# UmaimaKhan01/SkyEye-Aerial-Object-Detection-using-Yolo

Hardware: AMD Instinct MI355X
Metric: frames/sec @1280x1280 + p50 latency, skyeye_s 1-GPU and skyeye_l 8-GPU (higher is better)
Workload: dtype bf16

## Files before the change

skyeye-aerial-object-detection-using-yolo_amd/csrc/engine.cpp:

```cpp
#include "../../include/skyeye_hip.h"
#include "sky_kernels.h"
#include "build_hash.h"

#include <cstddef>
#include <hip/hip_runtime.h>

#include <algorithm>
#include <cmath>
#include <cstdio>
#include <cstring>
#include <map>
#include <memory>
#include <stdexcept>
#include <string>
#include <vector>

namespace sky {

struct Error : std::runtime_error {
    int code;
    Error(int c, const std::string& m) : std::runtime_error(m), code(c) {}
};

#define SKY_HIP(expr)                                                                                   \
// ... 1911 lines not shown

int sky_num_params(const sky_handle* h) { return h ? (int)h->e.spec.size() : 0; }

int sky_param_info(const sky_handle* h, int index, const char** name, int32_t* ndim, int64_t shape[4])
{
    if (!h || index < 0 || index >= (int)h->e.spec.size()) return SKY_ERR_INVALID;
    const ParamSpec& p = h->e.spec[index];
    if (name) *name = p.name.c_str();
    if (ndim) *ndim = (int32_t)p.shape.size();
    if (shape) for (size_t i = 0; i < 4; ++i) shape[i] = i < p.shape.size() ? p.shape[i] : 0;
    return SKY_OK;
}

int sky_load_weights(sky_handle* h, const sky_tensor_desc* descs, int n)
{
    if (!h) return SKY_ERR_INVALID;
    return guarded(h, [&] {
        for (int i = 0; i < n; ++i) {
            const sky_tensor_desc& d = descs[i];
            if (!d.name || !d.data) throw Error(SKY_ERR_INVALID, "sky_load_weights: null name/data");
            HostTensor t;
            for (int k = 0; k < d.ndim; ++k) t.shape.push_back(d.shape[k]);
            t.data.assign((const float*)d.data, (const float*)d.data + t.numel());
            h->e.weights[d.name] = std::move(t);
        }
        h->e.weights_dirty = true;
    });
}

int sky_plan(sky_handle* h, int n_inputs, const sky_buffer* in)
{
    if (!h) return SKY_ERR_INVALID;
    return guarded(h, [&] {
        if (n_inputs < 1 || n_inputs > SKY_MAX_IO) throw Error(SKY_ERR_INVALID, "sky_plan: bad input count");
        int ndev = 0;
        if (hipGetDeviceCount(&ndev) != hipSuccess || ndev == 0) throw Error(SKY_ERR_NO_DEVICE, "no HIP device visible: the HIP engine cannot run (there is no CPU fallback)");
        DeviceGuard dg(h->e.cfg.device);
        const Geometry g = geometry_of(n_inputs, in);
        plan(h->e, g);
        h->geom = g;
    });
}

int sky_num_outputs(const sky_handle* h) { return h ? (int)h->e.out_info.size() : 0; }

int sky_output_info(const sky_handle* h, int index, int32_t* ndim, int64_t shape[5])
{
    if (!h || index < 0 || index >= (int)h->e.out_info.size()) return SKY_ERR_INVALID;
    const IoInfo& io = h->e.out_info[index];
    if (ndim) *ndim = io.ndim;
    if (shape) for (int i = 0; i < 5; ++i) shape[i] = io.shape[i];
    return SKY_OK;
}

static void check_forward(sky_handle* h, int n_inputs, const sky_buffer* inputs, int n_outputs, const sky_buffer* outputs)
{
    if (!h->e.planned) throw Error(SKY_ERR_STATE, "sky_forward before sky_plan");
    if (h->e.weights_dirty) throw Error(SKY_ERR_STATE, "weights changed after sky_plan: call sky_plan again");
    if (!h->e.calibrated) throw Error(SKY_ERR_STATE, "fp8 engine without activation scales: call sky_calibrate (or sky_scales_write) after sky_plan");
    if (n_inputs != h->geom.n) throw Error(SKY_ERR_SHAPE, "sky_forward: input count differs from the plan");
    if (n_outputs != (int)h->e.out_info.size()) throw Error(SKY_ERR_SHAPE, "sky_forward: expected " + std::to_string(h->e.out_info.size()) + " outputs");
    for (int i = 0; i < n_inputs; ++i) {
        if (!inputs[i].data) throw Error(SKY_ERR_INVALID, "sky_forward: null input");
        for (int k = 0; k < h->geom.ndim[i]; ++k)
            if (inputs[i].shape[k] != h->geom.shape[i][k]) throw Error(SKY_ERR_SHAPE, "sky_forward: input shape differs from the plan");
    }
    std::vector<char> optional(n_outputs, 0);
    for (const Op& op : h->e.ops)
        if (op.kind == OP_CONV && op.head && op.raw_ext >= 16 && op.raw_ext - 16 < n_outputs) optional[op.raw_ext - 16] = 1;
    for (int i = 0; i < n_outputs; ++i) {
        if (!outputs[i].data && !optional[i]) throw Error(SKY_ERR_INVALID, "sky_forward: null output");
        if (!outputs[i].data) continue;
        const IoInfo& oi = h->e.out_info[i];
        bool same = outputs[i].ndim == oi.ndim;
        for (int k = 0; same && k < oi.ndim; ++k) same = outputs[i].shape[k] == oi.shape[k];
        if (!same) throw Error(SKY_ERR_SHAPE, "sky_forward: output " + std::to_string(i) + " has another shape than the plan's (sky_output_info)");
    }
}

int sky_forward(sky_handle* h, int n_inputs, const sky_buffer* inputs, int n_outputs, const sky_buffer* outputs, void* stream)
{
    if (!h) return SKY_ERR_INVALID;
    return guarded(h, [&] {
        check_forward(h, n_inputs, inputs, n_outputs, outputs);
        DeviceGuard dg(h->e.cfg.device);
        run(h->e, inputs, n_inputs, outputs, n_outputs, (hipStream_t)stream);
    });
}

int sky_time_forward(sky_handle* h, int n_inputs, const sky_buffer* inputs, int n_outputs, const sky_buffer* outputs, void* stream,
                     int iters, float* ms_per_iter)
{
    if (!h) return SKY_ERR_INVALID;
    return guarded(h, [&] {
        check_forward(h, n_inputs, inputs, n_outputs, outputs);
        DeviceGuard dg(h->e.cfg.device);
        hipStream_t s = (hipStream_t)stream;
        hipEvent_t e0, e1;
        SKY_HIP(hipEventCreate(&e0));
        SKY_HIP(hipEventCreate(&e1));
        SKY_HIP(hipEventRecord(e0, s));
        for (int i = 0; i < iters; ++i) run(h->e, inputs, n_inputs, outputs, n_outputs, s);
        SKY_HIP(hipEventRecord(e1, s));
        SKY_HIP(hipEventSynchronize(e1));
        float ms = 0;
        SKY_HIP(hipEventElapsedTime(&ms, e0, e1));
        (void)hipEventDestroy(e0);
        (void)hipEventDestroy(e1);
        if (ms_per_iter) *ms_per_iter = ms / (float)std::max(iters, 1);
    });
}

int sky_profile_forward(sky_handle* h, int n_inputs, const sky_buffer* inputs, int n_outputs, const sky_buffer* outputs, void* stream,
                        int iters, int max_ops, float* ms_per_op, double* flops_per_op, int32_t* tag_per_op, int32_t* n_ops)
{
    if (!h) return SKY_ERR_INVALID;
    return guarded(h, [&] {
        check_forward(h, n_inputs, inputs, n_outputs, outputs);
        DeviceGuard dg(h->e.cfg.device);
        const int n = (int)h->e.ops.size();
        if (n_ops) *n_ops = n;
        if (n > max_ops) throw Error(SKY_ERR_INVALID, "sky_profile_forward: max_ops too small");
        hipStream_t s = (hipStream_t)stream;
        std::vector<hipEvent_t> ev(n + 1);
        for (auto& e : ev) SKY_HIP(hipEventCreate(&e));
        std::vector<double> acc(n, 0.0);
        for (int it = 0; it < iters; ++it) {
            run(h->e, inputs, n_inputs, outputs, n_outputs, s, ev.data());
            SKY_HIP(hipEventSynchronize(ev[n]));
            for (int i = 0; i < n; ++i) {
                float ms = 0;
                SKY_HIP(hipEventElapsedTime(&ms, ev[i], ev[i + 1]));
                acc[i] += ms;
            }
        }
        for (auto& e : ev) (void)hipEventDestroy(e);
        for (int i = 0; i < n; ++i) {
            const Op& op = h->e.ops[i];
            if (ms_per_op) ms_per_op[i] = (float)(acc[i] / std::max(iters, 1));
            if (flops_per_op) flops_per_op[i] = op.flops;
            if (tag_per_op) tag_per_op[i] = (int)op.kind * 10000 + (op.kind == OP_CONV || op.kind == OP_IMPORT ? op.variant : 0);
        }
    });
}

int sky_op_info(const sky_handle* h, int index, char* text, int text_len)
{
    if (!h || !text || index < 0 || index >= (int)h->e.ops.size()) return SKY_ERR_INVALID;
    static const char* names[] = {"import", "export", "conv", "maxpool5", "upsample", "ca_reduce", "ca_mlp", "sa_stats", "sa_gate", "scale", "decode", "layernorm", "attention", "cla", "export_tokens"};
    const Op& op = h->e.ops[index];
    if (op.kind == OP_CONV)
        snprintf(text, text_len, "conv %dx%d s%d %d->%d in %dx%dx%d out %dx%d ld %d/%d%s%s%s %s%d", op.ks, op.ks, op.stride, op.cin, op.cout,
                 op.in.B, op.in.H, op.in.W, op.Ho, op.Wo, op.in.ld, op.out.ld, op.res.valid() ? (op.in2_cin ? " +res in2" : " +res") : (op.in2_cin ? " in2" : ""), op.up2 ? " up2" : "",
                 op.head ? " head" : "", op.variant >= 9000 ? "fused-into-previous" : op.variant >= 8500 ? "csp-stage-fused-" : op.variant >= 8000 ? "stem+stride2-fused-" : op.variant == 1628 ? "cv3+head/" : op.variant == 3256 ? "gemm1x1/" : op.variant == 7128 ? "bneck" : op.variant == 7256 ? "bneck128x2/" : op.variant == 7257 ? "bneck128x2-fp8/" : op.variant == 7065 ? "bneck64x3/" : op.variant == 7066 ? "bneck64x4-fp8/" : op.variant >= 7000 ? "halo-cv1+3x3-" : op.variant >= 6000 ? "halo-s2-" : op.variant >= 5000 ? "halo-narrow" : op.variant >= 4600 ? "deep3x3/" : op.variant >= 4000 ? "halo" : op.variant >= 3000 ? "ring" : op.variant >= 2000 ? "stream" : op.variant >= 1500 ? "head-stream" : "tile", op.variant % (op.variant >= 1500 && op.variant < 2000 ? 500 : 1000));
    else
        snprintf(text, text_len, "%s in %dx%dx%dx%d out C%d", names[op.kind], op.in.B, op.in.H, op.in.W, op.in.C, op.out.C);
    if (h->e.opts) {
        const size_t n = strlen(text);
        if ((int)n + 16 < text_len) snprintf(text + n, text_len - n, " opts=0x%x", h->e.opts);
    }
    return SKY_OK;
}

int sky_op_bytes(const sky_handle* h, int index, double* bytes)
{
    if (!h || !bytes || index < 0 || index >= (int)h->e.ops.size()) return SKY_ERR_INVALID;
    const Op& op = h->e.ops[index];
    const int es = h->e.esize();
    auto sz = [&](const TV& t, int esz) { return (t.buf >= 0 || t.ext >= 0) && t.B ? (double)t.B * t.H * t.W * t.C * (t.buf >= 0 ? dtype_size(t.dt) : esz) : 0.0; };
    double b = sz(op.in, es) + sz(op.out, es) + sz(op.res, es) + sz(op.in2, es);
    if (op.kind == OP_CONV && op.head) b += 2.0 * op.in.B * op.Ho * op.Wo * (double)op.cout * 4;
    if (op.kind == OP_IMPORT) b += (double)op.out.B * op.src_c * op.src_h * op.src_w;
    *bytes = b;
    return SKY_OK;
}

int sky_op_io_bytes(const sky_handle* h, int index, int with_raw, double* read_bytes, double* written_bytes)
{
    if (!h || !read_bytes || !written_bytes || index < 0 || index >= (int)h->e.ops.size()) return SKY_ERR_INVALID;
    const Op& op = h->e.ops[index];
    const int es = h->e.esize();
    auto sz = [&](const TV& t, int esz) { return (t.buf >= 0 || t.ext >= 0) && t.B ? (double)t.B * t.H * t.W * t.C * (t.buf >= 0 ? dtype_size(t.dt) : esz) : 0.0; };
    double r = sz(op.in, es) + sz(op.res, es) + sz(op.in2, es), w = sz(op.out, es);
    if (op.kind == OP_CONV && op.head) w += (with_raw ? 2.0 : 1.0) * op.in.B * op.Ho * op.Wo * (double)op.cout * 4;
    if (op.kind == OP_IMPORT) r = (double)op.out.B * op.src_c * op.src_h * op.src_w;
    *read_bytes = r;
    *written_bytes = w;
    return SKY_OK;
}

int sky_plan_stats(const sky_handle* h, double* flops, double* activation_bytes, double* weight_bytes, int32_t* launches)
{
    if (!h || !h->e.planned) return SKY_ERR_STATE;
    if (flops) *flops = h->e.flops;
    if (activation_bytes) *activation_bytes = h->e.act_bytes;
    if (weight_bytes) *weight_bytes = h->e.weight_bytes;
    if (launches) *launches = (int32_t)h->e.ops.size();
    return SKY_OK;
}

int sky_num_packed(const sky_handle* h)
{
    if (!h || !h->e.planned) return SKY_ERR_STATE;
    return (int)h->e.convs.size();
}

int sky_packed_info(const sky_handle* h, int i, sky_packed_desc* out)
{
    if (!h || !out) return SKY_ERR_INVALID;
    if (!h->e.planned) return SKY_ERR_STATE;
    if (i < 0 || i >= (int)h->e.convs.size()) return SKY_ERR_INVALID;
    const DevConv& d = h->e.convs[i];
    memset(out, 0, sizeof(*out));
    snprintf(out->name, sizeof(out->name), "%s", d.name.c_str());
    out->rows = d.rows; out->cout = d.cout; out->kpad = d.Kpad; out->kernel_size = d.ks; out->cin = d.cin;
    out->dtype = d.cdt;
    return SKY_OK;
}

int sky_packed_read(sky_handle* h, int i, void* weights_host, size_t weight_bytes, float* bias_host, size_t bias_count)
{
    if (!h) return SKY_ERR_INVALID;
    return guarded(h, [&] {
        if (!h->e.planned) throw Error(SKY_ERR_STATE, "sky_packed_read: plan the graph first (weights are packed at plan time)");
        DeviceGuard dg(h->e.cfg.device);
        if (i < 0 || i >= (int)h->e.convs.size()) throw Error(SKY_ERR_INVALID, "sky_packed_read: index out of range");
        const DevConv& d = h->e.convs[i];
        if (weights_host) {
            if (weight_bytes < d.bytes) throw Error(SKY_ERR_INVALID, "sky_packed_read: weight buffer too small");
            SKY_HIP(hipMemcpy(weights_host, d.w, d.bytes, hipMemcpyDeviceToHost));
        }
        if (bias_host) {
            if (bias_count < (size_t)d.rows) throw Error(SKY_ERR_INVALID, "sky_packed_read: bias buffer too small");
            SKY_HIP(hipMemcpy(bias_host, d.bias, (size_t)d.rows * sizeof(float), hipMemcpyDeviceToHost));
        }
    });
}

int sky_packed_scales(sky_handle* h, int i, float* scales_host, size_t count)
{
    if (!h) return SKY_ERR_INVALID;
    return guarded(h, [&] {
        if (!h->e.planned) throw Error(SKY_ERR_STATE, "sky_packed_scales: plan the graph first");
        if (i < 0 || i >= (int)h->e.convs.size() || !scales_host) throw Error(SKY_ERR_INVALID, "sky_packed_scales: bad argument");
        const DevConv& d = h->e.convs[i];
        if (count < (size_t)d.rows) throw Error(SKY_ERR_INVALID, "sky_packed_scales: buffer too small");
        for (int r = 0; r < d.rows; ++r) scales_host[r] = d.w_scale.empty() ? (float)(1.0 / (double)d.pre) : d.w_scale[r];
    });
}

int sky_calibrate(sky_handle* h, int n_inputs, const sky_buffer* inputs, void* stream)
{
    if (!h) return SKY_ERR_INVALID;
    return guarded(h, [&] {
        if (n_inputs != h->geom.n) throw Error(SKY_ERR_SHAPE, "sky_calibrate: input count differs from the plan");
        for (int i = 0; i < n_inputs; ++i)
            if (!inputs[i].data) throw Error(SKY_ERR_INVALID, "sky_calibrate: null input");
        DeviceGuard dg(h->e.cfg.device);
        calibrate(h->e, n_inputs, inputs, (hipStream_t)stream);
    });
}

int sky_num_scales(const sky_handle* h) { return h && h->e.planned ? (int)h->e.bufs.size() : 0; }

int sky_scales_read(sky_handle* h, float* scales_host, int n)
{
    if (!h) return SKY_ERR_INVALID;
    return guarded(h, [&] {
        if (!h->e.planned || !scales_host || n < (int)h->e.bufs.size()) throw Error(SKY_ERR_INVALID, "sky_scales_read: plan first / buffer too small");
        for (size_t i = 0; i < h->e.bufs.size(); ++i) {
            TV t; t.buf = (int)i; t.dt = h->e.bufs[i].dt;
            scales_host[i] = tv_scale(h->e, t);
        }
    });
}

int sky_scales_write(sky_handle* h, const float* scales_host, int n)
{
    if (!h) return SKY_ERR_INVALID;
    return guarded(h, [&] {
        if (!h->e.planned || !scales_host || n != (int)h->e.bufs.size()) throw Error(SKY_ERR_INVALID, "sky_scales_write: plan first; one scale per workspace buffer (sky_num_scales)");
        if (h->e.dtype != SKY_FP8) throw Error(SKY_ERR_STATE, "sky_scales_write: only the fp8 engine has activation scales");
        for (int i = 0; i < n; ++i)
            if (!(scales_host[i] > 0.0f)) throw Error(SKY_ERR_INVALID, "sky_scales_write: scales must be positive");
        DeviceGuard dg(h->e.cfg.device);
        for (int i = 0; i < n; ++i) {
            int r = i;
            while (h->e.bufs[r].tie >= 0) r = h->e.bufs[r].tie;
            if (h->e.bufs[i].dt == SKY_FP8) h->e.bufs[r].scale = scales_host[i];
        }
        apply_scales(h->e);
        h->e.calibrated = true;
    });
}

int sky_nms(sky_handle* h, const float* det, int B, int N, int nc, const sky_nms_params* p, float* out, int32_t* counts, void* stream)
{
    if (!h) return SKY_ERR_INVALID;
    return guarded(h, [&] {
        if (!det || !p || !out || !counts) throw Error(SKY_ERR_INVALID, "sky_nms: null argument");
        const bool has_strides = p->struct_size == sizeof(sky_nms_params);
        if (!has_strides && p->struct_size != offsetof(sky_nms_params, out_image_stride))
            throw Error(SKY_ERR_INVALID, "sky_nms: sky_nms_params size mismatch (ABI)");
        if (B < 1 || N < 1 || nc < 1) throw Error(SKY_ERR_SHAPE, "sky_nms: bad geometry");
        if (p->max_detections < 1 || p->max_detections > 4096) throw Error(SKY_ERR_INVALID, "sky_nms: max_detections must be in [1, 4096]");
        if (p->n_classes > 64) throw Error(SKY_ERR_INVALID, "sky_nms: at most 64 class filters");
        DeviceGuard dg(h->e.cfg.device);
// ... 129 lines not shown
```

skyeye-aerial-object-detection-using-yolo_amd/csrc/k_conv_halo.hip:

```cpp
#include "sky_kernels.h"

#ifndef SKY_HALO_VGPR
#define SKY_HALO_VGPR 256
#endif

#include "conv_frag.h"

#ifdef SKY_EXPERIMENTS
#define SKY_DBG(a) ((a).dbg)
#else
#define SKY_DBG(a) 0
#endif

#include <stdio.h>
#include <stdlib.h>

#include <type_traits>

namespace sky {

static constexpr int HWV = 4;

static constexpr int HPIX = 352;
static constexpr int HPL = HPIX * 32;
// ... 979 lines not shown
{
    constexpr int NB = NF * 16;
    const size_t lds = (size_t)3 * NB * 256 + 2 * 4 * SPL + (sizeof(T) == 1 ? 2 : 1) * NB * 4;
    auto kern = conv_halo_small_s2_kernel<T, NF, SQ, TO>;
    static size_t attr[16] = {0};
    {
        const hipError_t e = ensure_lds_attr(reinterpret_cast<const void*>(kern), lds, a.device, attr);
        if (e != hipSuccess) return e;
    }
    const int per_cu = (int)(160 * 1024 / lds) < 4 ? (int)(160 * 1024 / lds) : 4;
    const int ntile = a.B * ((a.Ho + a.tile_h - 1) / a.tile_h) * ((a.Wo + a.tile_w - 1) / a.tile_w);
    const int gy = a.Cout / NB;
    const int slots = per_cu * n_cu / gy > 0 ? per_cu * n_cu / gy : 1;
    const int gx = ntile < slots ? ntile : slots;
    kern<<<dim3(gx, gy), dim3(HWV * 64), lds, s>>>(a);
    return hipGetLastError();
}

template <typename T, typename TO>
static hipError_t halo_small_dispatch(int cb, int nb, const ConvArgs& a, hipStream_t s, int n_cu)
{
    const bool sq = a.tile_w == 16 && a.tile_h == 16;
    if (a.src_mode) {
        if constexpr (sizeof(T) >= 2) {
            constexpr int CBR = 16 * (int)sizeof(T);
            if (cb != CBR) return hipErrorNotSupported;
#define SKY_RAW(NFF, SQQ) (a.src_mode == 1 ? halo_small_launch<T, CBR, NFF, SQQ, 1, TO>(a, s, n_cu) : halo_small_launch<T, CBR, NFF, SQQ, 2, TO>(a, s, n_cu))
            if (nb == 32) return sq ? SKY_RAW(2, true) : SKY_RAW(2, false);
            return sq ? SKY_RAW(4, true) : SKY_RAW(4, false);
#undef SKY_RAW
        } else {
            return hipErrorNotSupported;
        }
    }
    if (cb == 32) {
        if (nb == 32) return sq ? halo_small_launch<T, 32, 2, true, 0, TO>(a, s, n_cu) : halo_small_launch<T, 32, 2, false, 0, TO>(a, s, n_cu);
        return sq ? halo_small_launch<T, 32, 4, true, 0, TO>(a, s, n_cu) : halo_small_launch<T, 32, 4, false, 0, TO>(a, s, n_cu);
    }
    if (nb == 32) return sq ? halo_small_launch<T, 64, 2, true, 0, TO>(a, s, n_cu) : halo_small_launch<T, 64, 2, false, 0, TO>(a, s, n_cu);
    return sq ? halo_small_launch<T, 64, 4, true, 0, TO>(a, s, n_cu) : halo_small_launch<T, 64, 4, false, 0, TO>(a, s, n_cu);
}

static bool halo_types_ok(int dtype, const ConvArgs& a, bool narrow)
{
    const int odt = a.out_dt < 0 ? dtype : a.out_dt;
    return odt == dtype || (dtype == 1 && odt == 2 && (narrow || a.stride == 2));
}

static bool halo_small_ok(int dtype, ConvArgs& a)
{
    const int esz = dtype_size(dtype);
    if (a.ks != 3 || a.stride != 1 || a.pad != 1 || a.head || a.out_f32 || a.up2) return false;
    if (!halo_types_ok(dtype, a, true)) return false;
    if ((!a.src_mode && a.in_bytes == 0) || a.out_bytes == 0 || (a.res && a.res_bytes == 0)) return false;
    const long cb = (long)a.Cin * esz;
    if (!((cb == 32 || cb == 64) && (a.Cout == 32 || a.Cout % 64 == 0))) return false;
    if ((long)a.Kpad * esz < 9L * a.Cin * esz || (long)a.Cout * a.Kpad * esz >= (1L << 31)) return false;
    if (a.opts & OPT_HALO_OFF) return false;
    const double cover = pick_tile(a, SPX);
    return (a.opts & OPT_HALO_FORCE) || cover >= 0.75;
}

bool conv_accepts_raw(int dtype, const ConvArgs& a0)
{
    if (a0.opts & OPT_NO_FUSED_IMPORT) return false;
    if (dtype == 2) return false;
    ConvArgs a = a0;
    a.src_mode = 1;
    return a.Cin == 16 && !a.res && halo_small_ok(dtype, a) && a.tile_w == 16 && a.tile_h == 16 && a.W % 2 == 0;
}

static bool cv1_shape_ok(int dtype, ConvArgs& a)
{
    if (dtype == 2)
        return (a.Cin == 128 && a.Cout == 128 && bneck128w8_shape_ok(a)) || (a.Cin == 64 && a.Cout == 64 && bneck64w8_shape_ok(a));
    if (dtype != 1 || (a.out_dt >= 0 && a.out_dt != 1)) return false;
    if (a.ks != 3 || a.stride != 1 || a.pad != 1 || a.head || a.out_f32 || a.up2 || a.src_mode || a.f2_w) return false;
    if (a.Cin == 128 && a.Cout == 128) return bneck128w_shape_ok(a) || bneck128_shape_ok(a);
    if (a.Cin != 64 || a.Cout != 64 || a.c1_Kpad < 64) return false;
    if (bneck64w_shape_ok(a)) return true;
    if (a.in_bytes == 0 || a.out_bytes == 0) return false;
    if ((long)a.Kpad * 2 < 9L * 128 || (a.opts & (OPT_HALO_OFF | OPT_NO_FUSE_CV1))) return false;
    const double cover = pick_tile(a, HPIX);
    return (a.opts & OPT_HALO_FORCE) || cover >= 0.75;
}

bool conv_accepts_cv1(int dtype, const ConvArgs& a0)
{
    ConvArgs a = a0;
    return cv1_shape_ok(dtype, a);
}

hipError_t launch_conv_halo(int dtype, const ConvArgs& a0, hipStream_t s, int* variant, int* fused)
{
    ConvArgs a = a0;
    if (a.c1_w) {
        if (!cv1_shape_ok(dtype, a)) return hipErrorInvalidValue;
        if (dtype == 2) {
            const hipError_t e8 = a.Cin == 64 ? launch_bneck64w8(a, s) : launch_bneck128w8(a, s);
            if (e8 == hipSuccess && variant) *variant = a.Cin == 64 ? 7066 : 7257;
            return e8 == hipErrorNotSupported ? hipErrorInvalidValue : e8;
        }
        if (a.Cin == 128) {
            if (bneck128w_shape_ok(a)) {
                const hipError_t ew = launch_bneck128w(a, s);
                if (ew == hipSuccess && variant) *variant = 7256;
                return ew;
            }
            const hipError_t e0 = launch_bneck128(a, s);
            if (e0 == hipSuccess && variant) *variant = 7128;
            return e0;
        }
        if (bneck64w_shape_ok(a)) {
            const hipError_t e6 = launch_bneck64w(a, s);
            if (e6 == hipSuccess && variant) *variant = 7065;
            return e6;
        }
        const int n_cu1 = a.n_cu > 0 ? a.n_cu : 256;
        const bool sq1 = a.tile_w == 16 && a.tile_h == 16;
        const hipError_t e1 = sq1 ? halo_launch<__bf16, 4, true, false, 0, __bf16, true>(a, s, n_cu1) : halo_launch<__bf16, 4, false, false, 0, __bf16, true>(a, s, n_cu1);
        if (e1 == hipSuccess && variant) *variant = 7064;
        return e1;
    }
    const int n_cu = a.n_cu > 0 ? a.n_cu : 256;
    const int esz = dtype_size(dtype);
    const int odt = a.out_dt < 0 ? dtype : a.out_dt;
    if (a.ks != 3 || (a.stride != 1 && a.stride != 2) || a.pad != 1 || a.head || a.out_f32 || a.up2) return hipErrorNotSupported;
    if ((!a.src_mode && a.in_bytes == 0) || a.out_bytes == 0 || (a.res && a.res_bytes == 0)) return hipErrorNotSupported;
    const long cb = (long)a.Cin * esz;
    const bool small = a.stride == 1 && (cb == 32 || cb == 64) && (a.Cout == 32 || a.Cout % 64 == 0);
    const bool small_s2 = a.stride == 2 && cb == 64 && (a.Cout == 32 || a.Cout % 64 == 0) && !a.src_mode && !a.f2_w;
    if (!halo_types_ok(dtype, a, small || small_s2)) return hipErrorNotSupported;
    if (small_s2) {
        if ((long)a.Kpad * esz < 9L * a.Cin * esz || (long)a.Cout * a.Kpad * esz >= (1L << 31)) return hipErrorNotSupported;
        if (!(a.opts & OPT_HALO_FORCE)) return hipErrorNotSupported;
        pick_tile(a, SPX);
        const bool sq2 = a.tile_w == 16 && a.tile_h == 16;
        hipError_t e2;
#define SKY_S2(T, TO) (a.Cout == 32 ? (sq2 ? halo_small_s2_launch<T, 2, true, TO>(a, s, n_cu) : halo_small_s2_launch<T, 2, false, TO>(a, s, n_cu)) \
                                    : (sq2 ? halo_small_s2_launch<T, 4, true, TO>(a, s, n_cu) : halo_small_s2_launch<T, 4, false, TO>(a, s, n_cu)))
        if (dtype == 0) e2 = SKY_S2(float, float);
        else if (dtype == 1 && odt == 1) e2 = SKY_S2(__bf16, __bf16);
        else if (dtype == 1) e2 = SKY_S2(__bf16, fp8_t);
        else e2 = SKY_S2(fp8_t, fp8_t);
#undef SKY_S2
        if (e2 == hipSuccess && variant) *variant = 6000 + (a.Cout == 32 ? 32 : 64);
        return e2;
    }
    if (!small && a.stride == 1 && conv3x3_deep_ok(dtype, a)) {
        const hipError_t ed = launch_conv3x3_deep(dtype, a, s);
        if (ed == hipSuccess && variant) *variant = 4600 + 128;
        return ed;
    }
    if (!small && (a.src_mode || cb % 128 != 0 || a.Cout % 64 != 0)) return hipErrorNotSupported;
    if ((long)a.Kpad * esz < 9L * a.Cin * esz) return hipErrorNotSupported;
    if ((long)a.Cout * a.Kpad * esz >= (1L << 31)) return hipErrorNotSupported;
    if (a.opts & OPT_HALO_OFF) return hipErrorNotSupported;
    {
        const int skip = (int)(a.opts >> OPT_SKIP_SHIFT) & 31;
        if (small ? (skip & 4) : (a.stride == 2 ? (skip & 2) : (skip & 1))) return hipErrorNotSupported;
        if (!small && ((a.Cout % 128 == 0) ? (skip & 8) : (skip & 16))) return hipErrorNotSupported;
    }
    if (!small && a.stride == 2) {
        if (a.opts & OPT_S2_OFF) return hipErrorNotSupported;
    }
    const double cover = pick_tile(a, small ? SPX : HPIX);
    if (!(a.opts & OPT_HALO_FORCE) && cover < 0.75) return hipErrorNotSupported;
    if (small) {
        const int nb = a.Cout == 32 ? 32 : 64;
        hipError_t e;
        if (dtype == 0) e = halo_small_dispatch<float, float>((int)cb, nb, a, s, n_cu);
        else if (dtype == 1 && odt == 1) e = halo_small_dispatch<__bf16, __bf16>((int)cb, nb, a, s, n_cu);
        else if (dtype == 1) e = halo_small_dispatch<__bf16, fp8_t>((int)cb, nb, a, s, n_cu);
        else e = halo_small_dispatch<fp8_t, fp8_t>((int)cb, nb, a, s, n_cu);
        if (e == hipSuccess && variant) *variant = 5000 + nb;
        return e;
    }
    const int nb = (a.Cout % 128 == 0 && !(a.opts & OPT_NF8_OFF) && dtype != 0) ? 128 : 64;
    const bool sq = a.tile_w == 16 && a.tile_h == 16;
    hipError_t e;
#define SKY_HALO(T, S2V) (nb == 128 ? (sq ? halo_launch<T, 8, true, S2V>(a, s, n_cu) : halo_launch<T, 8, false, S2V>(a, s, n_cu)) \
                                    : (sq ? halo_launch<T, 4, true, S2V>(a, s, n_cu) : halo_launch<T, 4, false, S2V>(a, s, n_cu)))
    if (a.stride == 2 && dtype == 1 && odt == 2) {
        e = nb == 128 ? (sq ? halo_launch<__bf16, 8, true, true, 0, fp8_t>(a, s, n_cu) : halo_launch<__bf16, 8, false, true, 0, fp8_t>(a, s, n_cu))
                      : (sq ? halo_launch<__bf16, 4, true, true, 0, fp8_t>(a, s, n_cu) : halo_launch<__bf16, 4, false, true, 0, fp8_t>(a, s, n_cu));
    } else if (a.stride == 2) {
        e = dtype == 0 ? SKY_HALO(float, true) : dtype == 1 ? SKY_HALO(__bf16, true) : SKY_HALO(fp8_t, true);
    } else if (dtype != 2 && a.f2_w && nb == 64 && a.Cout == 64 && a.f2_cin == 64 && a.f2_cout == 64 && a.f2_koff == 0 && a.f2_out_bytes) {
        if (dtype == 0) e = sq ? halo_launch<float, 4, true, false, 64>(a, s, n_cu) : halo_launch<float, 4, false, false, 64>(a, s, n_cu);
        else e = sq ? halo_launch<__bf16, 4, true, false, 64>(a, s, n_cu) : halo_launch<__bf16, 4, false, false, 64>(a, s, n_cu);
        if (e == hipSuccess && fused) *fused = 1;
    } else {
        e = dtype == 0 ? SKY_HALO(float, false) : dtype == 1 ? SKY_HALO(__bf16, false) : SKY_HALO(fp8_t, false);
    }
#undef SKY_HALO
    if (e == hipSuccess && variant) *variant = (a.stride == 2 ? 6000 : 4000) + nb;
    return e;
}

}
```

skyeye-aerial-object-detection-using-yolo_amd/csrc/sky_kernels.h:

```cpp
#pragma once
#include <hip/hip_runtime.h>
#include <stdint.h>

namespace sky {

enum Act { ACT_NONE = 0, ACT_SILU = 1, ACT_RELU = 2 };

enum PlanOpt : unsigned {
    OPT_HALO_OFF = 1u << 0,
    OPT_HALO_FORCE = 1u << 1,
    OPT_NF8_OFF = 1u << 2,
    OPT_NF8_SOLO = 1u << 3,
    OPT_S2_OFF = 1u << 4,
    OPT_NO_STREAM = 1u << 5,
    OPT_NO_RING = 1u << 6,
    OPT_OLDGRID = 1u << 7,
    OPT_NO_FUSED_IMPORT = 1u << 8,
    OPT_FUSE = 1u << 9,
    OPT_NO_SPP_PYRAMID = 1u << 10,
    OPT_ATTN_VALU = 1u << 11,
    OPT_NO_FUSE_CV1 = 1u << 12,
    OPT_NO_STEM_DOWN = 1u << 13,
    OPT_NO_WINATTN = 1u << 14,
    OPT_NO_CSP_STAGE = 1u << 15,
    OPT_NO_HEAD_STREAM = 1u << 21,
    OPT_HEAD_STREAM_FORCE = 1u << 22,
    OPT_NO_BNECK128 = 1u << 23,
    OPT_NO_DEEP3X3 = 1u << 24,
    OPT_NO_IN2 = 1u << 25,
    OPT_NO_CV3_HEAD = 1u << 26,
    OPT_NO_GEMM1X1 = 1u << 27,
    OPT_GEMM1X1_FORCE = 1u << 28,
    OPT_BNECK128_SOLO = 1u << 29,
    OPT_BNECK_PAIR = 1u << 30,
    OPT_NO_BNECK64W = 1u << 31,
    OPT_SKIP_SHIFT = 16,
};

inline hipError_t ensure_lds_attr(const void* kern, size_t lds, int device, size_t (&state)[16])
{
    const int d = device >= 0 && device < 16 ? device : 0;
    if (lds <= state[d] && state[d] != 0) return hipSuccess;
    const hipError_t e = hipFuncSetAttribute(kern, hipFuncAttributeMaxDynamicSharedMemorySize, (int)lds);
    if (e == hipSuccess) state[d] = lds;
    return e;
}

struct ConvArgs {
    const void* in;
    const void* w;
    const float* bias;
    void* out;
    const void* res;
    const void* zero;
    int B, H, W, Cin, ldi;
    int Ho, Wo, Cout, ldo, ldr;
    int ks, stride, pad;
    int Kpad;
    int act;
    int up2;
    int out_f32;
    int M;
    int ntiles;
    int cpt_shift;
    int tile_w, tile_h;
    unsigned magic_w, magic_h;
    int dbg;
    const float* mult;
    float out_inv_scale, res_scale;
    int out_dt;
    unsigned opts;
    int device, n_cu;
    int src_mode;
    const void* f2_w;
    const float* f2_bias;
    void* f2_out;
    int f2_cin, f2_cout, f2_ldo, f2_act, f2_Kpad, f2_koff;
    unsigned f2_out_bytes;
    const void* c1_w;
    const float* c1_bias;
    int c1_Kpad, c1_res;
    const float* c1_mult;
    float c1_out_inv_scale;
    unsigned out_bytes, res_bytes;
    unsigned in_bytes;
    const void* in2;
    int in2_cin, ldi2, in2_up2;
    unsigned in2_bytes;
    int head;
    float* raw;
    float* det;
    int na, no;
    long det_rows;
    long det_off;
    float stride_px;
    float anchor_wh[16];
};

#if defined(__HIPCC__)
template <bool FAST>
__device__ __forceinline__ float head_sigmoid(float v)
{
    if (FAST) return __builtin_amdgcn_rcpf(1.0f + __builtin_amdgcn_exp2f(v * -1.4426950408889634f));
    return 1.0f / (1.0f + expf(-v));
}
#endif

inline int dtype_size(int dtype) { return dtype == 0 ? 4 : dtype == 1 ? 2 : 1; }
int conv_pick_bn(int cout);
size_t conv_weight_rows(int cout);
int conv_k_step(int dtype);
hipError_t launch_conv(int dtype, const ConvArgs& a, hipStream_t s, int* variant = nullptr, int* fused = nullptr);
hipError_t launch_conv_stream(int dtype, const ConvArgs& a, hipStream_t s, int* variant = nullptr, int* fused = nullptr);
hipError_t launch_conv_halo(int dtype, const ConvArgs& a, hipStream_t s, int* variant = nullptr, int* fused = nullptr);
bool conv_accepts_raw(int dtype, const ConvArgs& a);
bool conv_accepts_in2(int dtype, const ConvArgs& a);
bool conv_accepts_cv1(int dtype, const ConvArgs& a);

struct StemDownArgs {
    const unsigned char* frames;
    int B, Hr, Wr;
    const void* w1;
    const float* bias1;
    int kpad1;
    const void* w2;
    const float* bias2;
    int kpad2;
    void* out;
    int Ho, Wo, ldo;
    int c1, c2;
    unsigned opts;
    int device, n_cu;
};
bool stem_down_supported(const StemDownArgs& a);
hipError_t launch_stem_down(const StemDownArgs& a, hipStream_t s);

struct CspStageArgs {
    const void* in;
    int ldi;
    unsigned in_bytes;
    void* out;
    int ldo;
    int B, H, W, c, hidden;
    const void* w12;
    const void* wb1;
    const void* wb2;
    const void* w3;
    const float *b12, *bb1, *bb2, *b3;
    int kpad12, kpadb1, kpadb2, kpad3;
    int shortcut;
    unsigned opts;
    int device, n_cu;
};
bool cv3_head_supported(int dtype, const ConvArgs& a);
hipError_t launch_cv3_head(int dtype, const ConvArgs& a, hipStream_t s);
bool gemm1x1_ok(int dtype, const ConvArgs& a);
hipError_t launch_gemm1x1(int dtype, const ConvArgs& a, hipStream_t s, int* variant);
bool head_stream_supported(int dtype, const ConvArgs& a);
hipError_t launch_head_stream(int dtype, const ConvArgs& a, hipStream_t s, int* variant);

bool bneck128_shape_ok(const ConvArgs& a);
hipError_t launch_bneck128(const ConvArgs& a, hipStream_t s);
bool bneck64w_shape_ok(const ConvArgs& a);
hipError_t launch_bneck64w(const ConvArgs& a, hipStream_t s);
bool bneck64w8_shape_ok(const ConvArgs& a);
hipError_t launch_bneck64w8(const ConvArgs& a, hipStream_t s);
bool bneck128w8_shape_ok(const ConvArgs& a);
hipError_t launch_bneck128w8(const ConvArgs& a, hipStream_t s);
bool bneck128w_shape_ok(const ConvArgs& a);
hipError_t launch_bneck128w(const ConvArgs& a, hipStream_t s);

bool conv3x3_deep_ok(int dtype, const ConvArgs& a);
hipError_t launch_conv3x3_deep(int dtype, const ConvArgs& a, hipStream_t s);

bool csp_stage_supported(const CspStageArgs& a);
hipError_t launch_csp_stage(const CspStageArgs& a, hipStream_t s);

hipError_t launch_import(int dtype, const void* src, int src_u8, int src_nhwc, void* dst, int B, int C, int H, int W,
                         int Cpad, int ld, int s2d, int scale255, hipStream_t s, float out_inv_scale = 1.0f);
hipError_t launch_export(int dtype, const void* src, int ld, float* dst, int B, int C, int H, int W, hipStream_t s, float in_scale = 1.0f);
hipError_t launch_amax(int dtype, const void* x, int ld, long pixels, int C, unsigned int* amax, hipStream_t s);
hipError_t launch_spp_pyramid(int dtype, const void* src, int lds_, void* dst, int ldd, int B, int H, int W, int C, int level_stride,
                              hipStream_t s);
hipError_t launch_maxpool5(int dtype, const void* src, int lds_, void* dst, int ldd, int B, int H, int W, int C,
                           hipStream_t s);
hipError_t launch_upsample(int dtype, const void* src, int lds_, void* dst, int ldd, int B, int H, int W, int C, int Ho,
                           int Wo, hipStream_t s);

hipError_t launch_letterbox(const unsigned char* src, int H0, int W0, unsigned char* dst, int H1, int W1, int nh, int nw, int top, int left,
                            int pad, int chw, int rev, hipStream_t s);

hipError_t launch_decode(int dtype, const float* raw, float* det, int B, int na, int gh, int gw, int no, long det_rows, long det_off,
                         float stride_px, const float* anchor_wh , hipStream_t s);

hipError_t launch_ca_reduce(int dtype, const void* x, int ld, int B, int HW, int C, int nchunk, float* part,
                            hipStream_t s, float in_scale = 1.0f);
hipError_t launch_ca_mlp(const float* part, int B, int HW, int C, int nchunk, int R, const float* w0, const float* w2,
                         float* att, hipStream_t s);
hipError_t launch_sa_stats(int dtype, const void* x, int ld, const float* att, int B, int HW, int C, float* stats,
                           hipStream_t s, float in_scale = 1.0f);
hipError_t launch_sa_gate(const float* stats, const float* w, int B, int H, int W, float* gate, hipStream_t s);
hipError_t launch_scale(int dtype, const void* x, int ldx, const float* att, const float* gate, void* out, int ldo,
                        int B, int HW, int C, hipStream_t s, float in_scale = 1.0f, float out_inv_scale = 1.0f);

hipError_t launch_layernorm(int dtype, const void* x, int ldx, void* y, int ldy, const float* g, const float* b, long tokens, int C,
                            hipStream_t s);
hipError_t launch_attention(int dtype, const void* qkv, int ldq, void* out, int ldo, int G, int N, int C, int heads, float scale,
                            const float* bias, const float* mask, int nW, int ws, int mh, int mw, hipStream_t s, unsigned opts = 0);
hipError_t launch_cla(int dtype, const void* q, int ldq, const void* kv, int ldkv, int v_off, float* scores, void* out, int ldo, int B, int H,
                      int W, int h, int w, int C, int heads, float scale, float r2, hipStream_t s);
hipError_t launch_export_tokens(int dtype, const void* src, int ld, float* dst, long tokens, int C, hipStream_t s);

struct NmsArgs {
    const float* det;
    int B, N, nc;
    float conf, iou, max_wh;
    int agnostic, multi_label, max_det, max_nms, mode;
    int n_classes;
    int classes[64];
    float* out;
    int* counts;
    long out_stride;
    long counts_stride;
    int* blk_counts;
    int* totals;
    unsigned long long* keys;
    unsigned long long* keys2;
    float* cand;
    long cap;
    int device;
};
size_t nms_workspace_bytes(int B, int N, int nc, int multi_label, long* cap_out);
hipError_t launch_nms(const NmsArgs& a, hipStream_t s);
hipError_t launch_box_iou(const float* box1, int n, int box1_4xn, const float* box2, int m, float* out, hipStream_t s);

hipError_t launch_scale_img(const void* src, int src_u8, int planes, int H, int W, float* dst, int sh, int sw, int PH, int PW, int flip, float pad,
                            hipStream_t s);
hipError_t launch_map_detections(const float* src, int B, int N, int no, int row0, int rows, float scale, int flip, float img_h, float img_w,
                                 const int* origins, int tpi, float* dst, long dst_rows, long dst_row0, hipStream_t s);
hipError_t launch_offset_boxes(float* rows, const int* counts, int T, int R, int cols, const int* origins, hipStream_t s);
hipError_t launch_tile_gather(const unsigned char* src, int H0, int W0, int src_chw, const int* origins, int n, unsigned char* dst, int th, int tw,
                              int pad, int rev, hipStream_t s);

}
```

Baseline: 7729.

## Add dedicated pipelined stride-2 3x3 conv kernel for deep bf16 layers

Adds a new persistent kernel for stride-2 3x3 convolutions with wide output channels (multiples of 256). It double-buffers weight slabs and phase-split input halos through direct buffer-to-LDS loads, with tap ordering arranged so loads overlap the matrix instructions. The halo dispatcher routes eligible non-small stride-2 layers to it before the generic halo path. This trades extra kernel complexity and a fixed 16x16-style tiling for less memory-stall time on the downsampling convs in the backbone.

```diff
diff --git a/skyeye-aerial-object-detection-using-yolo_amd/csrc/engine.cpp b/skyeye-aerial-object-detection-using-yolo_amd/csrc/engine.cpp
--- a/skyeye-aerial-object-detection-using-yolo_amd/csrc/engine.cpp
+++ b/skyeye-aerial-object-detection-using-yolo_amd/csrc/engine.cpp
@@ -2087,7 +2087,7 @@
     if (op.kind == OP_CONV)
         snprintf(text, text_len, "conv %dx%d s%d %d->%d in %dx%dx%d out %dx%d ld %d/%d%s%s%s %s%d", op.ks, op.ks, op.stride, op.cin, op.cout,
                  op.in.B, op.in.H, op.in.W, op.Ho, op.Wo, op.in.ld, op.out.ld, op.res.valid() ? (op.in2_cin ? " +res in2" : " +res") : (op.in2_cin ? " in2" : ""), op.up2 ? " up2" : "",
-                 op.head ? " head" : "", op.variant >= 9000 ? "fused-into-previous" : op.variant >= 8500 ? "csp-stage-fused-" : op.variant >= 8000 ? "stem+stride2-fused-" : op.variant == 1628 ? "cv3+head/" : op.variant == 3256 ? "gemm1x1/" : op.variant == 7128 ? "bneck" : op.variant == 7256 ? "bneck128x2/" : op.variant == 7257 ? "bneck128x2-fp8/" : op.variant == 7065 ? "bneck64x3/" : op.variant == 7066 ? "bneck64x4-fp8/" : op.variant >= 7000 ? "halo-cv1+3x3-" : op.variant >= 6000 ? "halo-s2-" : op.variant >= 5000 ? "halo-narrow" : op.variant >= 4600 ? "deep3x3/" : op.variant >= 4000 ? "halo" : op.variant >= 3000 ? "ring" : op.variant >= 2000 ? "stream" : op.variant >= 1500 ? "head-stream" : "tile", op.variant % (op.variant >= 1500 && op.variant < 2000 ? 500 : 1000));
+                 op.head ? " head" : "", op.variant >= 9000 ? "fused-into-previous" : op.variant >= 8500 ? "csp-stage-fused-" : op.variant >= 8000 ? "stem+stride2-fused-" : op.variant == 1628 ? "cv3+head/" : op.variant == 3256 ? "gemm1x1/" : op.variant == 7128 ? "bneck" : op.variant == 7256 ? "bneck128x2/" : op.variant == 7257 ? "bneck128x2-fp8/" : op.variant == 7065 ? "bneck64x3/" : op.variant == 7066 ? "bneck64x4-fp8/" : op.variant >= 7000 ? "halo-cv1+3x3-" : op.variant >= 6600 ? "s2deep/" : op.variant >= 6000 ? "halo-s2-" : op.variant >= 5000 ? "halo-narrow" : op.variant >= 4600 ? "deep3x3/" : op.variant >= 4000 ? "halo" : op.variant >= 3000 ? "ring" : op.variant >= 2000 ? "stream" : op.variant >= 1500 ? "head-stream" : "tile", op.variant % (op.variant >= 1500 && op.variant < 2000 ? 500 : 1000));
     else
         snprintf(text, text_len, "%s in %dx%dx%dx%d out C%d", names[op.kind], op.in.B, op.in.H, op.in.W, op.in.C, op.out.C);
     if (h->e.opts) {
diff --git a/skyeye-aerial-object-detection-using-yolo_amd/csrc/k_conv3x3_s2.hip b/skyeye-aerial-object-detection-using-yolo_amd/csrc/k_conv3x3_s2.hip
--- /dev/null
+++ b/skyeye-aerial-object-detection-using-yolo_amd/csrc/k_conv3x3_s2.hip
@@ -0,0 +1,305 @@
+#include "sky_kernels.h"
+
+#include "conv_frag.h"
+
+namespace sky {
+
+namespace s2 {
+constexpr int NW = 8, NT = NW * 64;
+constexpr int TS = 16, HWD = TS + 2;
+constexpr int XPIX = 352, PL = XPIX * 32, CHB = 4 * PL;
+constexpr int XDMA = XPIX / 32;
+constexpr int MAXC = 512;
+constexpr int lds_bytes(int NB) { return 2 * CHB + 2 * NB * 128 + MAXC * 4; }
+static_assert(lds_bytes(256) <= 160 * 1024, "one workgroup per CU");
+
+static __device__ __forceinline__ void dma16(__amdgpu_buffer_rsrc_t rsrc, char* dst, int voff, int soff)
+{
+    __builtin_amdgcn_raw_ptr_buffer_load_lds(rsrc, (__attribute__((address_space(3))) void*)dst, 16, voff, soff, 0, 0);
+}
+static __device__ __forceinline__ void barrier()
+{
+    __builtin_amdgcn_s_barrier();
+    asm volatile("" ::: "memory");
+}
+template <int N>
+static __device__ __forceinline__ void wait_vm()
+{
+    static_assert(N >= 0 && N < 64, "vmcnt is a 6-bit counter");
+    asm volatile("s_waitcnt vmcnt(%0) lgkmcnt(0)" ::"n"(N) : "memory");
+}
+static __device__ __forceinline__ void wait_n(int n)
+{
+    switch (n) {
+    case 5: wait_vm<5>(); break;
+    case 6: wait_vm<6>(); break;
+    case 8: wait_vm<8>(); break;
+    case 16: wait_vm<16>(); break;
+    default: wait_vm<0>(); break;
+    }
+}
+constexpr int tap_of(int q) { return (int)((0x453718620ull >> (4 * q)) & 15); }
+constexpr int phase_of(int q) { return q < 4 ? 0 : q < 6 ? 1 : q < 8 ? 2 : 3; }
+}
+
+template <int NB, bool SQ>
+__global__ void __launch_bounds__(s2::NT) conv3x3_s2_kernel(const ConvArgs a)
+{
+    using namespace s2;
+    constexpr int SLAB = NB * 128;
+    constexpr int WP = NB / 64;
+    constexpr int JW = NB / 32, HG = JW / 2;
+    extern __shared__ __attribute__((aligned(1024))) char smem[];
+    char* const himg = smem;
+    char* const ring = smem + 2 * CHB;
+    float* const lbias = reinterpret_cast<float*>(ring + 2 * SLAB);
+
+    const int tid = threadIdx.x, lane = tid & 63, wave = __builtin_amdgcn_readfirstlane(tid >> 6);
+    const int fr = lane & 15, fq = lane >> 4;
+    const int hc = wave & 1, pg = wave >> 1;
+    const int tw = SQ ? TS : a.tile_w, th = SQ ? TS : a.tile_h, hpw = tw + 2;
+    const int tiles_x = (a.Wo + tw - 1) / tw, tiles_y = (a.Ho + th - 1) / th;
+    const int gy = a.Cout / NB;
+    const int nitem = a.B * tiles_y * tiles_x * gy;
+    int item, tstep, tend;
+    tile_walk(nitem, item, tstep, tend);
+    if (item >= tend) return;
+    const int pix_b = a.ldi * 2;
+    const int Cb = a.Cin * 2;
+    const int nchunk = Cb >> 7;
+    const int wpitch = a.Kpad * 2;
+
+    for (int i = tid; i < a.Cout; i += NT) lbias[i] = a.bias[i];
+
+    const __amdgpu_buffer_rsrc_t irsrc = __builtin_amdgcn_make_buffer_rsrc(const_cast<void*>(a.in), 0, (int)a.in_bytes, 0x00020000);
+    const __amdgpu_buffer_rsrc_t orsrc = __builtin_amdgcn_make_buffer_rsrc(a.out, 0, (int)a.out_bytes, 0x00020000);
+    const __amdgpu_buffer_rsrc_t wrsrc = __builtin_amdgcn_make_buffer_rsrc(const_cast<void*>(a.w), 0, (int)((long)a.Cout * wpitch), 0x00020000);
+
+    int wrel[WP];
+#pragma unroll
+    for (int q = 0; q < WP; ++q) {
+        const int row = (wave * WP + q) * 8 + (lane >> 3);
+        const int c = (lane & 7) ^ ((row >> 1) & 7);
+        const int j = (row >> 4) & 7, r = row & 15;
+        const int ch = (row >> 7) * 128 + (j >> 1) * 32 + (r >> 2) * 8 + (j & 1) * 4 + (r & 3);
+        wrel[q] = ch * wpitch + c * 16;
+    }
+    auto issue_slab = [&](int n0, int chunk, int tap, int stage) {
+        char* const dst = ring + stage * SLAB + wave * (WP * 1024);
+        const int soff = n0 * wpitch + tap * Cb + chunk * 128;
+#pragma unroll
+        for (int q = 0; q < WP; ++q) dma16(wrsrc, dst + q * 1024, wrel[q], soff);
+    };
+    auto decode_item = [&](int it, int& bimg, int& y0, int& x0, int& n0) {
+        const int t = it / gy;
+        n0 = (it - t * gy) * NB;
+        const int tx = t % tiles_x;
+        const int q = t / tiles_x;
+        bimg = q / tiles_y;
+        y0 = (q - bimg * tiles_y) * th;
+        x0 = tx * tw;
+    };
+    auto issue_img = [&](int bimg, int y0, int x0, int chunk, int ph, int buf) {
+        const int ry0 = 2 * (y0 - 1) + (ph < 2), rx0 = 2 * (x0 - 1) + ((ph & 1) == 0);
+        const int base = ((bimg * a.H + ry0) * a.W + rx0) * pix_b + chunk * 128 + (wave & 3) * 16;
+        char* const dst = himg + buf * CHB + (wave & 3) * PL;
+        int ln = lane;
+        asm volatile("" : "+v"(ln));
+        const int b0 = wave < 4 ? 0 : 6, b1 = wave < 4 ? 6 : XDMA;
+        for (int b = b0; b < b1; ++b) {
+            const int p = b * 32 + (ln >> 1);
+            const int hy = SQ ? (p * 3641) >> 16 : (int)(((unsigned)p * a.magic_h) >> 16), hx = p - hy * hpw;
+            const int kk = (ln & 1) ^ ((p >> 3) & 1);
+            const bool ok = hy <= th && hx <= tw && (unsigned)(ry0 + 2 * hy) < (unsigned)a.H && (unsigned)(rx0 + 2 * hx) < (unsigned)a.W;
+            dma16(irsrc, dst + b * 1024, ok ? base + (2 * hy * a.W + 2 * hx) * pix_b + kk * 64 : -1, 0);
+        }
+    };
+
+    const int arow = fr * 128 + ((fq ^ ((fr >> 1) & 7)) << 4);
+    int pb[SQ ? 10 : 4];
+    if constexpr (SQ) {
+#pragma unroll
+        for (int c = 0; c < 10; ++c) pb[c] = fq * PL + ((4 * pg) * HWD + fr) * 32 + (((fr + 8 * pg + c) & 8) << 1);
+    } else {
+#pragma unroll
+        for (int i = 0; i < 4; ++i) {
+            const int idx = pg * 64 + i * 16 + fr;
+            int ty = (int)(((unsigned)idx * a.magic_w) >> 16);
+            const int tx = idx - ty * tw;
+            if (ty >= th) ty = -1;
+            pb[i] = fq * PL + (ty < 0 ? 0 : ty * hpw + tx) * 32;
+        }
+    }
+    auto pfrag = [&](int buf, int i, int oy, int ox, int kk) -> u32x4_t {
+        if constexpr (SQ) {
+            const int r = i + oy;
+            int q = pb[2 * r + ox];
+            if (kk) {
+                asm volatile("" : "+v"(q));
+                q ^= 16;
+            }
+            return *reinterpret_cast<const u32x4_t*>(himg + q + (buf * CHB + (r * HWD + ox) * 32));
+        } else {
+            const int A = pb[i] + (oy * hpw + ox) * 32;
+            const int q = A + (((A >> 8) & 1) << 4);
+            return *reinterpret_cast<const u32x4_t*>(himg + buf * CHB + (kk ? q ^ 16 : q));
+        }
+    };
+
+    int bimg, y0, x0, n0;
+    decode_item(item, bimg, y0, x0, n0);
+    asm volatile("s_waitcnt lgkmcnt(0)" ::: "memory");
+    barrier();
+    int stg = 0;
+    issue_slab(n0, 0, tap_of(0), 0);
+    issue_img(bimg, y0, x0, 0, 0, 0);
+    bool first = true;
+
+    for (;;) {
+        const int next = item + tstep;
+        const bool has_next = next < tend;
+        int nb = 0, ny0 = 0, nx0 = 0, nn0 = 0;
+        if (has_next) decode_item(next, nb, ny0, nx0, nn0);
+        f32x4_t acc[JW][4];
+        {
+            int fqb = fq;
+            asm volatile("" : "+v"(fqb));
+#pragma unroll
+            for (int j = 0; j < JW; ++j) {
+                const f32x4_t c = *reinterpret_cast<const f32x4_t*>(lbias + n0 + (NB / 2) * hc + (j >> 1) * 32 + fqb * 8 + (j & 1) * 4);
+#pragma unroll
+                for (int i = 0; i < 4; ++i) acc[j][i] = c;
+            }
+        }
+
+        for (int c = 0; c < nchunk; ++c) {
+            const bool last_chunk = c == nchunk - 1;
+#pragma unroll
+            for (int q = 0; q < 9; ++q) {
+                const int tap = tap_of(q), ph = phase_of(q), buf = ph & 1;
+                const int ky = (tap * 11) >> 5, kx = tap - ky * 3;
+                const int oy = ky != 0, ox = kx != 0;
+                int n = 0;
+                if (q == 1 || q == 5 || q == 7) n = wave < 4 ? 6 : 5;
+                if (q == 0 && c == 0 && !first) n = 4 * HG;
+                wait_n(n);
+                barrier();
+                if (q < 8) issue_slab(n0, c, tap_of(q + 1), stg ^ 1);
+                else if (!last_chunk) issue_slab(n0, c + 1, tap_of(0), stg ^ 1);
+                else if (has_next) issue_slab(nn0, 0, tap_of(0), stg ^ 1);
+                if (q == 0 || q == 4 || q == 6) issue_img(bimg, y0, x0, c, ph + 1, buf ^ 1);
+                else if (q == 8) {
+                    if (!last_chunk) issue_img(bimg, y0, x0, c + 1, 0, 0);
+                    else if (has_next) issue_img(nb, ny0, nx0, 0, 0, 0);
+                }
+                const char* const wb = ring + stg * SLAB + hc * (JW * 2048);
+                u32x4_t pf[2][4], wq[3][2];
+#pragma unroll
+                for (int i = 0; i < 4; ++i) pf[0][i] = pfrag(buf, i, oy, ox, 0);
+#pragma unroll
+                for (int g = 0; g < 2 * HG + 2; ++g) {
+                    if (g < 2 * HG) {
+                        const int kk = g / HG, sp = g % HG;
+#pragma unroll
+                        for (int h = 0; h < 2; ++h)
+                            wq[g % 3][h] = *reinterpret_cast<const u32x4_t*>(wb + (2 * sp + h) * 2048 + (kk ? arow ^ 64 : arow));
+                    }
+                    if (g == 0) {
+#pragma unroll
+                        for (int i = 0; i < 4; ++i) pf[1][i] = pfrag(buf, i, oy, ox, 1);
+                    }
+                    if (g >= 2) {
+                        const int gg = g - 2, kk = gg / HG, sp = gg % HG;
+#pragma unroll
+                        for (int h = 0; h < 2; ++h)
+#pragma unroll
+                            for (int i = 0; i < 4; ++i) S1<__bf16>::mma(wq[gg % 3][h], pf[kk][i], acc[2 * sp + h][i]);
+                    }
+                    __builtin_amdgcn_sched_barrier(0);
+                }
+                stg ^= 1;
+            }
+        }
+
+        {
+            int fre = fr, fqe = fq;
+            asm volatile("" : "+v"(fre), "+v"(fqe));
+            const int nl = n0 + (NB / 2) * hc + 8 * fqe;
+#pragma unroll
+            for (int i = 0; i < 4; ++i) {
+                int oy, ox;
+                if constexpr (SQ) {
+                    oy = y0 + 4 * pg + i;
+                    ox = x0 + fre;
+                } else {
+                    const int idx = pg * 64 + i * 16 + fre;
+                    const int ty = (int)(((unsigned)idx * a.magic_w) >> 16);
+                    oy = ty < th ? y0 + ty : a.Ho;
+                    ox = x0 + idx - ty * tw;
+                }
+                const bool ok = oy < a.Ho && ox < a.Wo;
+                const int ooff = ok ? (((bimg * a.Ho + oy) * a.Wo + ox) * a.ldo + nl) * 2 : (int)0x80000000;
+#pragma unroll
+                for (int sp = 0; sp < HG; ++sp) {
+                    float v[8];
+#pragma unroll
+                    for (int e = 0; e < 8; ++e) {
+                        const float xx = e < 4 ? acc[2 * sp][i][e] : acc[2 * sp + 1][i][e - 4];
+                        v[e] = a.act == ACT_SILU ? S1<__bf16>::silu(xx) : xx;
+                    }
+                    Out8<__bf16>::store(Out8<__bf16>::pack(v, 1.0f), orsrc, ooff + sp * 64);
+                }
+            }
+        }
+        if (!has_next) break;
+        item = next; bimg = nb; y0 = ny0; x0 = nx0; n0 = nn0;
+        first = false;
+    }
+}
+
+bool conv3x3_s2_ok(int dtype, const ConvArgs& a)
+{
+    if (dtype != 1 || (a.out_dt >= 0 && a.out_dt != 1)) return false;
+    if (a.ks != 3 || a.stride != 2 || a.pad != 1 || a.head || a.up2 || a.out_f32 || a.src_mode || a.f2_w || a.c1_w || a.res) return false;
+    if (a.Ho != (a.H + 1) / 2 || a.Wo != (a.W + 1) / 2) return false;
+    if (a.Cin % 64 != 0 || a.Cout % 128 != 0 || a.Cout > s2::MAXC || (a.act != ACT_SILU && a.act != ACT_NONE)) return false;
+    if (a.ldi % 8 != 0 || a.ldo % 8 != 0) return false;
+    if (a.in_bytes == 0 || a.out_bytes == 0) return false;
+    if ((long)a.Kpad < 9L * a.Cin || (long)a.Cout * a.Kpad * 2 >= (1L << 31)) return false;
+    if (a.opts & (OPT_HALO_OFF | OPT_NO_DEEP3X3 | OPT_S2_OFF)) return false;
+    if (((a.opts >> OPT_SKIP_SHIFT) & 31) & 2) return false;
+    if (a.tile_w < 1 || a.tile_h < 1 || a.tile_w * a.tile_h > 256 || (a.tile_w + 2) * (a.tile_h + 2) > s2::XPIX) return false;
+    if (a.tile_w + 1 > 64 || a.magic_w != 65536u / (unsigned)a.tile_w + 1u || a.magic_h != 65536u / (unsigned)(a.tile_w + 2) + 1u) return false;
+    if (a.Cout % 256 != 0 && !(a.opts & OPT_HALO_FORCE)) return false;
+    const int th = (a.Ho + a.tile_h - 1) / a.tile_h, tw = (a.Wo + a.tile_w - 1) / a.tile_w;
+    const double cover = (double)a.Ho * a.Wo / ((double)th * tw * 256.0);
+    return (a.opts & OPT_HALO_FORCE) || cover >= 0.75;
+}
+
+template <int NB, bool SQ>
+static hipError_t s2_launch(const ConvArgs& a, hipStream_t s)
+{
+    static size_t attr[16] = {0};
+    {
+        const hipError_t e = ensure_lds_attr(reinterpret_cast<const void*>(conv3x3_s2_kernel<NB, SQ>), s2::lds_bytes(NB), a.device, attr);
+        if (e != hipSuccess) return e;
+    }
+    const int nitem = a.B * ((a.Ho + a.tile_h - 1) / a.tile_h) * ((a.Wo + a.tile_w - 1) / a.tile_w) * (a.Cout / NB);
+    const int n_cu = a.n_cu > 0 ? a.n_cu : 256;
+    const int gx = nitem < n_cu ? nitem : n_cu;
+    auto kern = conv3x3_s2_kernel<NB, SQ>;
+    hipLaunchKernelGGL(kern, dim3(gx), dim3(s2::NT), s2::lds_bytes(NB), s, a);
+    return hipGetLastError();
+}
+
+hipError_t launch_conv3x3_s2(int dtype, const ConvArgs& a, hipStream_t s, int* nb)
+{
+    if (!conv3x3_s2_ok(dtype, a)) return hipErrorNotSupported;
+    const bool sq = a.tile_w == 16 && a.tile_h == 16;
+    const int n = a.Cout % 256 == 0 ? 256 : 128;
+    if (nb) *nb = n;
+    if (n == 256) return sq ? s2_launch<256, true>(a, s) : s2_launch<256, false>(a, s);
+    return sq ? s2_launch<128, true>(a, s) : s2_launch<128, false>(a, s);
+}
+
+}
diff --git a/skyeye-aerial-object-detection-using-yolo_amd/csrc/k_conv_halo.hip b/skyeye-aerial-object-detection-using-yolo_amd/csrc/k_conv_halo.hip
--- a/skyeye-aerial-object-detection-using-yolo_amd/csrc/k_conv_halo.hip
+++ b/skyeye-aerial-object-detection-using-yolo_amd/csrc/k_conv_halo.hip
@@ -1155,6 +1155,16 @@
         if (ed == hipSuccess && variant) *variant = 4600 + 128;
         return ed;
     }
+    if (!small && a.stride == 2) {
+        ConvArgs at = a;
+        pick_tile(at, HPIX);
+        if (conv3x3_s2_ok(dtype, at)) {
+            int nbd = 0;
+            const hipError_t e2d = launch_conv3x3_s2(dtype, at, s, &nbd);
+            if (e2d == hipSuccess && variant) *variant = 6600 + nbd;
+            return e2d;
+        }
+    }
     if (!small && (a.src_mode || cb % 128 != 0 || a.Cout % 64 != 0)) return hipErrorNotSupported;
     if ((long)a.Kpad * esz < 9L * a.Cin * esz) return hipErrorNotSupported;
     if ((long)a.Cout * a.Kpad * esz >= (1L << 31)) return hipErrorNotSupported;
diff --git a/skyeye-aerial-object-detection-using-yolo_amd/csrc/sky_kernels.h b/skyeye-aerial-object-detection-using-yolo_amd/csrc/sky_kernels.h
--- a/skyeye-aerial-object-detection-using-yolo_amd/csrc/sky_kernels.h
+++ b/skyeye-aerial-object-detection-using-yolo_amd/csrc/sky_kernels.h
@@ -172,6 +172,8 @@
 
 bool conv3x3_deep_ok(int dtype, const ConvArgs& a);
 hipError_t launch_conv3x3_deep(int dtype, const ConvArgs& a, hipStream_t s);
+bool conv3x3_s2_ok(int dtype, const ConvArgs& a);
+hipError_t launch_conv3x3_s2(int dtype, const ConvArgs& a, hipStream_t s, int* nb);
 
 bool csp_stage_supported(const CspStageArgs& a);
 hipError_t launch_csp_stage(const CspStageArgs& a, hipStream_t s);
```

Result: no change. 7790 (median of 6 runs) (+0.8%).
